# SensorsINI/Control_Toolkit

Hardware: AMD Instinct MI355X
Metric: trajectory-steps/sec (N*H per controller.step) (higher is better)
Workload: dtype f32; 1 GPU; MPPI N=1024 global (1024 per GPU), H=50, period=1, predictor ODE (4 states, 1 input) [mppi_cfg2]; boundary=controller_mpc.step (Python; s in, u out on the host), samples=buffer, global_rollouts=1024, parallelism=single GPU

## Files before the change

### control_toolkit_amd/Optimizers/optimizer_mppi_hip.py

```python
from typing import Tuple

import numpy as np

from . import template_optimizer, logging_kwargs
from ..computation_library import HipLibrary


class optimizer_mppi_hip(template_optimizer):
    supported_computation_libraries = (HipLibrary,)
    engine_name = "mppi"

    def __init__(self, predictor, cost_function, control_limits: "Tuple[np.ndarray, np.ndarray]",
                 computation_library, seed, cc_weight: float, R: float, LBD: float, mpc_horizon: int,
                 num_rollouts: int, NU: float, SQRTRHOINV: float, period_interpolation_inducing_points: int,
                 optimizer_logging: bool, calculate_optimal_trajectory: bool = False, **kwargs):
        super().__init__(predictor=predictor, cost_function=cost_function, control_limits=control_limits,
                         optimizer_logging=optimizer_logging, seed=seed, num_rollouts=num_rollouts,
                         mpc_horizon=mpc_horizon, computation_library=computation_library,
                         calculate_optimal_trajectory=calculate_optimal_trajectory,
                         rng_mode=kwargs.get("rng_mode", "device"), device=kwargs.get("device", 0), **logging_kwargs(kwargs))
        self.cc_weight, self.R, self.LBD, self.NU = cc_weight, R, LBD, NU
        self._SQRTRHOINV = SQRTRHOINV
        self.period_interpolation_inducing_points = period_interpolation_inducing_points
        self.global_rollout_offset = int(kwargs.get("global_rollout_offset", 0))
        self.resident_idle_us = float(kwargs.get("resident_idle_us", 0.0) or 0.0)

    def configure(self, num_states: int, num_control_inputs: int, dt: float, predictor_specification: str, **kwargs):
        super().configure(num_states=num_states, num_control_inputs=num_control_inputs, default_configure=False)
        self._build_engine(dt, predictor_specification, cc_weight=self.cc_weight, R=self.R, LBD=self.LBD, NU=self.NU,
                           SQRTRHOINV=self._SQRTRHOINV,
                           period_interpolation_inducing_points=self.period_interpolation_inducing_points,
                           global_rollout_offset=self.global_rollout_offset)
        self.number_of_interpolation_inducing_points = self.engine.inducing_points()
        if self.resident_idle_us > 0.0:
            self.engine.resident_enable(True, self.resident_idle_us)
        self.optimizer_reset()

    def step(self, s: np.ndarray, time=None):
        fast = self._fast
        if fast is not None:
            u = fast(s)
            if u is not NotImplemented:
                return u
        if self.optimizer_logging:
            self.logging_values = {"s_logged": np.asarray(s).copy()}
        s = self._prepare_state(s)
        self._sync_parameters()
        noise = self._draws("normal", [self.num_rollouts, self.number_of_interpolation_inducing_points, self.num_control_inputs])
        self._publish_u(self.engine.step(s, noise, u_prev=self._u_prev()))
        self._lazy.clear()
# ... 14 lines not shown
```

### control_toolkit_amd/_capi.py

```python
from __future__ import annotations

import ctypes as C
import os
from types import SimpleNamespace
from typing import NamedTuple, Optional

import numpy as np

_HERE = os.path.dirname(os.path.abspath(__file__))
_LIB_NAME = "libctk_hip.so"
_lib = None

OPTIMIZERS = {"mppi": 0, "cem": 1, "rpgd": 2, "random_action": 3, "gradient": 4, "cem_naive_grad": 5,
              "cem_grad_bharadhwaj": 6, "cem_gmm": 7}
PREDICTORS = {"ODE": 0, "MLP": 1, "GRU": 2}
ENVIRONMENTS = {"CartPole": 0, "Quad2D": 1, "Hover": 2}
MAX_STATES, MAX_INPUTS = 8, 4
PARAMS = ("g", "m_cart", "m_pole", "L", "u_max", "M_fric", "J_fric", "target_position", "target_equilibrium",
          "dd_weight", "ep_weight", "ekp_weight", "cc_weight", "ccrc_weight", "R", "x_scale", "terminal_weight")
BUFFERS = {"Q": 0, "J": 1, "TRAJ": 2, "U_NOM": 3, "STD": 4, "ADAM_M": 5, "ADAM_V": 6, "AGES": 7, "BEST_IDX": 8, "PLAN": 9, "AGES_LOGGED": 10,
           "MIX_MU": 11, "MIX_STD": 12, "MIX_PROB": 13, "MIX_LABEL": 14}
LOC_NONE, LOC_HOST, LOC_DEVICE = 0, 1, 2
MLP_NUM_WEIGHTS = 1380

# ... 168 lines not shown

HYPERS = {"cc_weight": 0, "R": 1, "LBD": 2, "NU": 3, "SQRTRHOINV": 4}
_PROBLEM_HYPER = {
    "set_hyper": (C.c_int, [_H, C.c_int, C.c_void_p, C.c_int, C.c_void_p]),
    "get_hyper": (C.c_int, [_H, C.c_int, C.c_int, _FP]),
    "set_limits": (C.c_int, [_H, C.c_int, C.c_void_p, C.c_void_p, C.c_void_p]),
    "get_limits": (C.c_int, [_H, C.c_int, C.c_void_p, C.c_void_p]),
    "hypers_differ": (C.c_int, [_H]),
}
HYPER_SYMBOLS = {}
for _batch, _problem in _BATCH_FAMILIES[:3]:
    HYPER_SYMBOLS.update({f"{_problem}_{name}": sig for name, sig in _PROBLEM_HYPER.items()})
    HYPER_SYMBOLS[f"{_batch}_set_hyper"] = (C.c_int, [_H, C.c_int, C.c_float])


USER_ENVIRONMENTS = {}
ENV_USER = 3
_user_libs = {}


def load_library(path: str = None):
    global _lib
    if path is not None:
        if path not in _user_libs:
            _user_libs[path] = _bind_library(path)
        return _user_libs[path]
    if _lib is not None:
        return _lib
    try:
        import torch
# ... 4 lines not shown


def _bind_library(path: str):
    try:
        import torch
    except ImportError:
        pass
    if not os.path.exists(path):
        raise CtkError(f"{path} not found: build it with `make -C control_toolkit_amd/csrc` "
                       f"(or `python -c 'import __graft_entry__ as g; g.build()'`). There is no CPU fallback.")
    try:
        lib = C.CDLL(path)
    except OSError as e:
        raise CtkError(f"cannot load {path}: {e}") from e
    for name, (res, args) in list(SYMBOLS.items()) + list(RUN_SYMBOLS.items()) + list(EPISODE_SYMBOLS.items()) + list(LOOP_SYMBOLS.items()) + \
            list(GRU_LOOP_SYMBOLS.items()) + list(HYPER_SYMBOLS.items()):
        fn = getattr(lib, name)
        fn.restype, fn.argtypes = res, args
    if lib.ctk_abi_version() != 6:
        raise CtkError(f"{path}: ABI version mismatch")
    return lib


def environment_library(name: str):
    if name in ENVIRONMENTS:
        return load_library(), ENVIRONMENTS[name]
    if name in USER_ENVIRONMENTS:
        return load_library(USER_ENVIRONMENTS[name]), ENV_USER
    raise NotImplementedError(f"environment {name!r} is not built (have: {sorted(ENVIRONMENTS)} + registered user environments "
                              f"{sorted(USER_ENVIRONMENTS)}; control_toolkit_amd.build_env.register_environment compiles a model header)")

# ... 387 lines not shown
        if name == "BEST_IDX":
            return out.astype(np.int64)
        return out.reshape(shapes[name])

    def resident_enable(self, on: bool = True, idle_us: float = 200.0, read_ahead: bool = False):
        self._check(self._lib.ctk_resident_enable(self._h, (2 if read_ahead else 1) if on else 0, float(idle_us)))

    def resident_stop(self):
        self._check(self._lib.ctk_resident_stop(self._h))

    def resident_stats(self) -> dict:
        a, b, r, m = C.c_uint64(0), C.c_uint64(0), C.c_int(0), C.c_int(0)
        self._check(self._lib.ctk_resident_stats(self._h, C.byref(a), C.byref(b), C.byref(r), C.byref(m)))
        return {"launches": int(a.value), "steps": int(b.value), "running": bool(r.value), "mailbox": "device memory" if m.value else "pinned host memory"}

    def log_enable(self, capacity_steps: int):
        self._check(self._lib.ctk_log_enable(self._h, int(capacity_steps)))
        self.log_capacity = int(capacity_steps)

    def log_count(self) -> int:
        return int(self._lib.ctk_log_count(self._h))

    def log_read(self, name: str, first_step: int, n_steps: int) -> np.ndarray:
        N, H = self.N, self.H
        shape = {"Q": (N, H, self.C), "J": (N,), "TRAJ": (N, H + 1, self.S), "AGES": (N,)}[name]
        out = np.empty((int(n_steps),) + shape, np.float32)
        n = C.c_size_t()
        self._check(self._lib.ctk_log_read(self._h, BUFFERS[name], int(first_step), int(n_steps), _ptr(out), out.size, C.byref(n)))
        assert n.value == out.size
        return out
# ... 882 lines not shown
```

### control_toolkit_amd/csrc/ctk_api.hip

```cpp
#include <atomic>
#include <unordered_map>
#include <chrono>
#include <cmath>
#include <cstdio>
#include <cstring>
#include <string>
#include <vector>

#include "ctk_launch.h"
#include "ctk_host.h"
#include "ctk_device.h"
#include "ctk_mlp.h"
#include "ctk_gru.h"
#include "ctk_env.h"
#include "ctk_net.h"
#include <algorithm>
#include <cstdlib>

thread_local std::string ctk_host::g_create_error;
using namespace ctk_host;

namespace {

struct EventPair {
// ... 103 lines not shown
    CtkResidentBox* res_box_dev = nullptr;
    bool res_local = false;
    bool res_stream_isolated = false;
    CtkResidentStat* res_stat = nullptr;
    CtkResidentStat* res_stat_dev = nullptr;
    CtkResidentBox* d_res_relay = nullptr;
    void* d_res_args = nullptr;
    alignas(16) unsigned char res_args_host[CTK_RES_ARGS_BYTES];
    uint32_t res_req = 0;
    uint32_t res_relay_prime[2] = {0, 0};
    uint64_t res_launches = 0, res_steps = 0;
    std::string res_dominant_saved;
    std::unordered_map<const float*, const float*> res_follow;
    const float* res_prev_samples = nullptr;
    bool res_readahead = false;
    Owner own;
    ~ctk_handle();
};

namespace {

int fail(ctk_handle* h, int code, const std::string& msg) {
    if (h) h->err = msg; else g_create_error = msg;
    return code;
}

#define HIP_TRY(h, expr)                                                                      \
    do {                                                                                      \
        hipError_t _e = (expr);                                                               \
        if (_e != hipSuccess)                                                                 \
// ... 538 lines not shown
        }
        return fail(h, CTK_ERR_STATE, dev_err == 1 ? "timed out waiting for a peer's record (a rank is gone or out of step)"
                                                   : "in-launch record hand-off timed out (a workgroup's record never arrived)");
    }
    return h->log_cap ? log_step(h) : CTK_OK;
}

template <class F>
int guarded(ctk_handle* h, F&& body) {
    const uint32_t seq0 = h->seq;
    const int rc = body();
    if (rc != CTK_OK && h->seq == seq0) ++h->seq;
    return rc;
}

int resident_quiesce(ctk_handle* h) {
    if (!h->res_running) return CTK_OK;
    if (__atomic_load_n(&h->res_stat->state, __ATOMIC_ACQUIRE) != CTK_RES_LEFT) {
        volatile CtkResidentBox* b = h->res_box;
        b->cmd = CTK_RES_CMD_EXIT;
        b->tail = h->res_req + 1;
        __builtin_ia32_sfence();
        b->req = ++h->res_req;
        __builtin_ia32_sfence();
    }
    HIP_TRY(h, hipStreamSynchronize(h->stream));
    h->res_running = false;
    if (!h->res_dominant_saved.empty()) { h->dominant = h->res_dominant_saved; h->res_dominant_saved.clear(); }
    return CTK_OK;
}
// ... 62 lines not shown
                if (*slot == want) break;
                if (int rc = resident_launch(h, req)) return rc;
            }
            if (std::chrono::duration<double>(std::chrono::steady_clock::now() - t0).count() > 5.0) {
                (void)resident_quiesce(h);
                return fail(h, CTK_ERR_HIP, "resident step: no result within 5 s");
            }
        }
        __builtin_ia32_pause();
    }
    ++h->res_steps;
    h->cur ^= 1;
    return finish_step(h, u_out);
}

#define RES_Q(h) do { if ((h) != nullptr && (h)->res_running) { const int _q = resident_quiesce(h); if (_q != CTK_OK) return _q; } } while (0)

int check_predictor(ctk_handle* h) {
    if (h->cfg.predictor != CTK_PRED_ODE && !h->have_weights)
        return fail(h, CTK_ERR_STATE, "network predictor: call ctk_set_predictor_weights before stepping");
    return CTK_OK;
}

int mppi_block_parts(const ctk_handle* h) {
    if (h->generic && h->cfg.predictor != CTK_PRED_ODE) return ctk_g_rollout_net_blocks(h->env, h->net, CTK_G_MODE_MPPI, h->N, h->P, h->H);
    return h->generic ? ctk_g_rollout_blocks(h->N) : ctk_mppi_num_blocks(h->N, h->cfg.predictor);
}
bool mppi_env_kernel(const ctk_handle* h) {
    return h->generic && h->cfg.predictor == CTK_PRED_ODE && !ctk_mppi_uses_throughput_kernel(CTK_PRED_ODE, h->N) &&
           ctk_mppi_rollout_env_lds(h->env, h->P, h->H, h->N) <= 160 * 1024;
}
// ... 25 lines not shown
        if (h->cfg.predictor != CTK_PRED_ODE)
            HIP_TRY(h, ctk_launch_g_rollout_net(h->stream, h->env, h->net, CTK_G_MODE_MPPI, a, h->params, h->cfg.dt, h->cfg.intermediate_steps,
                                                h->mk, d_s, h->d_unom[h->cur], nullptr, 0, h->d_wperm, h->d_parts, log, ps.a, ps.b, &fz));
        else
            HIP_TRY(h, ctk_launch_g_rollout(h->stream, h->env, CTK_G_MODE_MPPI, a, h->params, h->cfg.dt, h->cfg.intermediate_steps, h->mk, d_s,
                                            h->d_unom[h->cur], nullptr, 0, h->d_parts, log, ps.a, ps.b));
        return CTK_OK;
    }
    const char* ran = nullptr;
    CTK_HSTAMP(h, 1);
    HIP_TRY(h, ctk_launch_mppi_rollout(h->stream, h->cfg.predictor, a, h->k, h->mk, d_s, h->d_unom[h->cur], h->d_wperm,
                                       h->d_parts, log, fz, ps.a, ps.b, &ran));
    CTK_HSTAMP(h, 2);
    if (ran != h->dominant_ran) { h->dominant_ran = ran; h->dominant = ran; }
    return CTK_OK;
}

int mppi_reduce_blocks(ctk_handle* h, const float** parts, int* n_parts) {
    int n = mppi_block_parts(h);
    const float* src = h->d_parts;
    float* bufs[2] = {h->d_parts2, h->d_parts3};
    int b = 0;
    while (n > 64) {
        HIP_TRY(h, ctk_launch_mppi_merge_partial(h->stream, src, n, 32, h->PC, h->mk.neg_inv_lbd, bufs[b]));
        n = (n + 31) / 32;
        src = bufs[b];
        b ^= 1;
    }
    *parts = src; *n_parts = n;
    return CTK_OK;
// ... 321 lines not shown
    return CTK_OK;
}

int fill_const(ctk_handle* h, float* d, float v, int n) {
    std::vector<float> tmp((size_t)n, v);
    HIP_TRY(h, hipMemcpyAsync(d, tmp.data(), n * sizeof(float), hipMemcpyHostToDevice, h->stream));
    HIP_TRY(h, hipStreamSynchronize(h->stream));
    return CTK_OK;
}

}

inline ctk_handle::~ctk_handle() {
    if (!stream && own.empty() && events.empty() && p2p_world == 0) return;
    hipSetDevice(cfg.device);
    (void)resident_quiesce(this);
    hipStreamSynchronize(stream);
    for (auto& e : events) { hipEventDestroy(e.a); hipEventDestroy(e.b); }
    ctk_p2p_close(this);
    own.release();
    if (own_stream && stream) hipStreamDestroy(stream);
}

extern "C" {

int ctk_abi_version(void) { return CTK_ABI_VERSION; }
static_assert(CTK_P_COUNT <= CTK_MAX_PARAMS && CTK_Q_COUNT <= CTK_MAX_PARAMS && CTK_V_COUNT <= CTK_MAX_PARAMS, "parameter table size");
static_assert(Env<CTK_ENV_QUAD2D>::S <= CTK_MAX_STATES && Env<CTK_ENV_QUAD2D>::C <= CTK_MAX_INPUTS, "environment dimensions");
static_assert(Env<CTK_ENV_HOVER>::S <= CTK_MAX_STATES && Env<CTK_ENV_HOVER>::C <= CTK_MAX_INPUTS, "environment dimensions");

// ... 159 lines not shown
    const bool gnet = generic && cfg->predictor != CTK_PRED_ODE;
    if (descends) h->dominant = gnet ? ctk_g_rpgd_descent_net_name(h->env, h->net, (int)N, (int)H) : generic ? ctk_g_rpgd_descent_name(h->env) : ctk_rpgd_descent_name(cfg->predictor, (int)N, (int)H);
    else {
        const int mode = cfg->optimizer == CTK_OPT_MPPI ? CTK_G_MODE_MPPI : CTK_G_MODE_AFFINE;
        h->dominant = gnet ? ctk_g_rollout_net_name(h->env, h->net, mode, mat, (int)N, (int)P, (int)H) : generic ? ctk_g_rollout_name(h->env, mode, mat)
                    : cfg->optimizer == CTK_OPT_MPPI ? ctk_mppi_rollout_name(cfg->predictor, mat, cfg->num_rollouts, cfg->period_interpolation_inducing_points == 1 && h->P == (int)H, false)
                                                     : ctk_affine_rollout_name(cfg->predictor, mat);
    }
    if (h->d_cem_ll && h->variant == CTK_OPT_CEM && cfg->cem_best_k <= (int)N) h->dominant = ctk_cem_fused_name(h->env, mat);
    if (cfg->optimizer == CTK_OPT_MPPI && mppi_env_kernel(h)) h->dominant = ctk_mppi_rollout_env_name(h->env, mat);
    if (!descends && cfg->optimizer != CTK_OPT_MPPI && affine_env_kernel(h) && !(h->d_cem_ll && h->variant == CTK_OPT_CEM)) h->dominant = ctk_affine_rollout_env_name(h->env, mat);
    if (h->gmm_in_rollout) h->dominant = ctk_affine_rollout_mix_name(h->env, mat);
    if (cfg->optimizer != CTK_OPT_RPGD)
        if (int rc = ctk_reset(h, nullptr, CTK_LOC_NONE)) { g_create_error = h->err; return rc; }
    HIP_CREATE(hipStreamSynchronize(h->stream));
    *out = made.release();
    return CTK_OK;
}

void ctk_destroy(ctk_handle* h) { delete h; }


int ctk_set_stream(ctk_handle* h, void* hip_stream) {
    RES_Q(h);
    if (!h) return CTK_ERR_INVALID_ARGUMENT;
    HIP_TRY(h, hipSetDevice(h->cfg.device));
    hipStream_t ns = (hipStream_t)hip_stream;
    if (ns == h->stream) return CTK_OK;
    if (h->own_stream && h->stream) {
        HIP_TRY(h, hipStreamSynchronize(h->stream));
// ... 172 lines not shown
    else HIP_TRY(h, hipMemsetAsync(gru_hidden(h), 0, GRU_HIDDEN_FLOATS * sizeof(float), h->stream));
    HIP_TRY(h, hipStreamSynchronize(h->stream));
    return CTK_OK;
}

size_t ctk_samples_needed(const ctk_handle* h) { return h ? samples_needed(h) : 0; }

int ctk_rng_get_position(const ctk_handle* h, uint32_t* call) {
    if (!h || !call) return CTK_ERR_INVALID_ARGUMENT;
    *call = h->call;
    return CTK_OK;
}

int ctk_rng_set_position(ctk_handle* h, uint32_t call) {
    if (!h) return CTK_ERR_INVALID_ARGUMENT;
    h->call = call;
    return CTK_OK;
}

int ctk_step(ctk_handle* h, const float* s, const float* u_prev, const float* samples, int samples_loc, float* u_out) {
    if (!h || !s) return h ? fail(h, CTK_ERR_INVALID_ARGUMENT, "ctk_step: NULL state") : CTK_ERR_INVALID_ARGUMENT;
    CTK_HSTAMP(h, 0);
    return guarded(h, [&]() -> int {
    if (h->mppi_pending) return fail(h, CTK_ERR_STATE, "ctk_step: a sharded step is pending (call ctk_mppi_step_end)");
    HIP_TRY(h, hipSetDevice(h->cfg.device));
    switch (h->cfg.optimizer) {
        case CTK_OPT_MPPI: {
            for (int i = 0; i < h->S; ++i) h->mppi_s[i] = s[i];
            if (resident_ok(h, samples_loc)) {
                const float* d_s = nullptr;
                if (int rc = resolve_samples(h, samples, samples_loc, (size_t)h->N * h->PC, &d_s)) return rc;
                return resident_step(h, s, u_prev, d_s, u_out);
            }
            if (int rc = resident_quiesce(h)) return rc;
            if (mppi_can_fuse(h)) {
                if (int rc = mppi_rollout(h, s, u_prev, samples, samples_loc, 1, nullptr)) return rc;
                h->cur ^= 1;
                if (int rc = mppi_advance_hidden(h)) return rc;
                return finish_step(h, u_out);
            }
            if (int rc = mppi_rollout(h, s, u_prev, samples, samples_loc, 0, nullptr)) return rc;
            const float* parts; int n_parts;
            if (int rc = mppi_reduce_blocks(h, &parts, &n_parts)) return rc;
            return mppi_update(h, parts, n_parts, u_out);
        }
        case CTK_OPT_CEM: return cem_step(h, s, u_prev, samples, samples_loc, u_out);
        case CTK_OPT_RANDOM_ACTION: return random_step(h, s, u_prev, samples, samples_loc, u_out);
        case CTK_OPT_RPGD: return rpgd_step(h, s, u_prev, samples, samples_loc, u_out);
    }
// ... 458 lines not shown
                HIP_TRY(h, hipStreamSynchronize(h->stream));
                (void)hipStreamDestroy(h->stream);
                h->stream = ns;
            }
        }
        (void)hipGetLastError();
        h->res_stream_isolated = true;
    }
    h->res_idle_us = idle_us;
    h->res_readahead = on == 2;
    h->res_follow.clear(); h->res_prev_samples = nullptr;
    h->res_enabled = true;
    return CTK_OK;
}

int ctk_resident_stop(ctk_handle* h) {
    if (!h) return CTK_ERR_INVALID_ARGUMENT;
    HIP_TRY(h, hipSetDevice(h->cfg.device));
    return resident_quiesce(h);
}

int ctk_resident_stats(const ctk_handle* h, uint64_t* launches, uint64_t* steps, int* running, int* mailbox_in_device_memory) {
    if (!h) return CTK_ERR_INVALID_ARGUMENT;
    if (h->res_stat && getenv("CTK_RES_TRACE"))
        fprintf(stderr, "[ctk resident] mailbox in %s memory; last request: fetch%s %.2f us, block 0's step %.2f us, inputs %s\n", h->res_local ? "device" : "pinned host",
                h->res_local ? "" : " + relay", (h->res_stat->t_relay & 0x7FFFFFFFu) * 0.01, h->res_stat->t_body * 0.01,
                (h->res_stat->t_relay & 0x80000000u) ? "prepared ahead" : "formed at the request");
    if (h->res_stat && getenv("CTK_RES_TRACE"))
    {
        fprintf(stderr, "[ctk resident] block 0's step: %u shader cycles -> %.0f MHz; stamps", h->res_stat->c_body, h->res_stat->c_body / (h->res_stat->t_body * 0.01 + 1e-9));
        for (int i = 1; i < 12; ++i) fprintf(stderr, " %d", (int)(h->res_stat->stamps[i] - h->res_stat->stamps[0]));
        fprintf(stderr, "\n");
    }
    if (launches) *launches = h->res_launches;
// ... 66 lines not shown
```

### control_toolkit_amd/csrc/ctk_launch.h

```cpp
#pragma once
#include <hip/hip_ext.h>
#include "ctk_common.h"

#define CTK_LAUNCH(kernel, grid, block, lds, st, e0, e1, ...)                                         \
    do {                                                                                              \
        if (e0) hipExtLaunchKernelGGL(kernel, grid, block, lds, st, e0, e1, 0, __VA_ARGS__);          \
        else hipLaunchKernelGGL(kernel, grid, block, lds, st, __VA_ARGS__);                           \
    } while (0)

#include <type_traits>
template <class F>
inline void ctk_with_bool(bool b, F&& f) {
    if (b) f(std::true_type{});
    else f(std::false_type{});
}

inline RolloutArgs ctk_rollout_args(const RolloutArgs& a_in, int C, int cols) {
    RolloutArgs a = a_in;
    a.C = C; a.P = cols; a.p_magic = ctk_magic_of(cols);
    return a;
}
inline RolloutArgs ctk_descent_args(const RolloutArgs& a_in, int C) {
    RolloutArgs a = a_in;
    a.C = C; a.p_magic = ctk_magic_of(a.H * C);
// ... 76 lines not shown
};
hipError_t ctk_launch_mppi_rollout(hipStream_t st, int pred, const RolloutArgs& a, const EnvK& k, const MppiK& m,
                                   const float* samples, const float* u_nom, const float* wperm, float* parts, bool log,
                                   const MppiFuse& fuse, hipEvent_t ev_start = nullptr, hipEvent_t ev_stop = nullptr,
                                   const char** ran = nullptr);
hipError_t ctk_launch_mppi_rollout_env(hipStream_t st, int env, const float* params, float dt, int isteps, const RolloutArgs& a, const MppiK& m,
                                       const float* samples, const float* u_nom, float* parts, bool log, const MppiFuse& fuse,
                                       hipEvent_t ev_start = nullptr, hipEvent_t ev_stop = nullptr);
size_t ctk_mppi_rollout_env_lds(int env, int P, int H, int N);
hipError_t ctk_launch_mppi_resident(hipStream_t st, int env, const float* params, float dt, int isteps, const RolloutArgs& a, const MppiK& m,
                                    float* u_nom0, float* u_nom1, float* parts, const MppiFuse& fuse, const CtkResidentBox* box_dev, int box_local,
                                    CtkResidentStat* stat_dev, CtkResidentBox* relay, double idle_us, uint32_t first_req, void* args_dev, void* args_host);
constexpr size_t CTK_RES_ARGS_BYTES = 1024;
const char* ctk_mppi_resident_name(int env, int N, int P);
const char* ctk_mppi_rollout_env_name(int env, bool log);
struct CtkBatchDesc {
    float* parts;
    unsigned long long* ll;
    float* J;
    float* Q_out;
    float* traj_out;
    float* unom[2];
    float* u_dev;
    float* u_host;
    uint32_t seed_lo, seed_hi;
};
struct CtkBatchStep {
    int32_t id;
    uint32_t seq;
    uint32_t call;
// ... 322 lines not shown
```

### control_toolkit_amd/csrc/ctk_mppi.hip

```cpp
#ifdef CTK_STAMPS
#define STAMP(i)                                                                                   \
    do {                                                                                           \
        __builtin_amdgcn_sched_barrier(0);                                                         \
        unsigned long long _t;                                                                     \
        asm volatile("s_memtime %0\n\ts_waitcnt lgkmcnt(0)" : "=s"(_t)::"memory");                 \
        __builtin_amdgcn_sched_barrier(0);                                                         \
        if (threadIdx.x == 0 && a.stamps) a.stamps[blockIdx.x * 16 + (i)] = _t;                     \
    } while (0)
#else
#define STAMP(i)
#endif

#include "ctk_rollout.h"
#include "ctk_env.h"
#include "ctk_mlp.h"
#include "ctk_gru.h"
#include "ctk_launch.h"
#include "ctk_mppi_merge.h"
#include <cstring>
#include <type_traits>

constexpr int MPPI_TRAJ = 64;
constexpr int MPPI_WAVES = 4;
constexpr int MPPI_BLOCK = MPPI_TRAJ * MPPI_WAVES;
// ... 1099 lines not shown
    ctk_with_bool(log, [&](auto log_c) {
        hipLaunchKernelGGL((ctk_mppi_batch_mlp_hp<decltype(log_c)::value>), grid, block, lds, st, desc_dev, steps_dev, a.interp, w_dev, k_dev, a.N, a.H,
                           a.P, pmagic, wstride, a, fz);
    });
}
static void launch_batch_gru_hp(hipStream_t st, dim3 grid, dim3 block, size_t lds, const CtkBatchDesc* desc_dev, const CtkBatchStep* steps_dev, const float* w_dev,
                                const unsigned char* k_dev, uint32_t pmagic, uint32_t wstride, const RolloutArgs& a,
                                const FuseArgs& fz, bool log, int form) {
    with_mppi_form<false>(form, [&](auto form_c) {
        ctk_with_bool(log, [&](auto log_c) {
            hipLaunchKernelGGL((ctk_mppi_batch_gru_hp<decltype(log_c)::value, decltype(form_c)::value>), grid, block, lds, st, desc_dev, steps_dev,
                               a.interp, w_dev, k_dev, a.N, a.H, a.P, pmagic, wstride, a, fz);
        });
    });
}
```

### include/ctk_hip.h

```cpp
#ifndef CTK_HIP_H
#define CTK_HIP_H

#include <stddef.h>
#include <stdint.h>

#ifdef __cplusplus
extern "C" {
#endif

#define CTK_ABI_VERSION 6
#define CTK_MAX_STATES 8
#define CTK_MAX_INPUTS 4

typedef struct ctk_handle ctk_handle;

typedef enum ctk_status {
    CTK_OK = 0,
    CTK_ERR_INVALID_ARGUMENT = 1,
    CTK_ERR_UNSUPPORTED = 2,
    CTK_ERR_HIP = 3,
    CTK_ERR_NO_DEVICE = 4,
    CTK_ERR_STATE = 5
} ctk_status;

// ... 297 lines not shown
int ctk_gru_problem_set_weights(ctk_gru_batch* b, int n_ids, const int32_t* ids, const float* w, size_t n);
int ctk_gru_problem_have_weights(const ctk_gru_batch* b, int problem);
int ctk_gru_problem_get_hidden(ctk_gru_batch* b, int n_ids, const int32_t* ids, float* dst);
int ctk_gru_problem_set_hidden(ctk_gru_batch* b, int n_ids, const int32_t* ids, const float* src);
int ctk_gru_batch_fit(int num_rollouts, int mpc_horizon, int period_interpolation_inducing_points, int* blocks, int* record_words,
                      int* wide_tail, size_t* lds_bytes);

#ifdef __cplusplus
}
#endif
#include "ctk_hip_run.h"
#include "ctk_hip_episode.h"
#include "ctk_hip_loop.h"
#include "ctk_hip_gru.h"
#include "ctk_hip_hyper.h"
#endif
```

Baseline: 2.704 billion trajectory-steps/s.

## Pre-launch next MPPI step kernel that waits on a device-memory mailbox

Adds a launch-ahead path. After each MPPI step, once calls keep arriving in quick succession, the host enqueues the next step's fused rollout kernel in advance. That kernel spins on a fine-grained VRAM mailbox (large-BAR) until the host writes the new state and u_prev, then runs. If no request arrives within a fuse window, the kernel exits and the host falls back to a normal launch. This is meant to hide kernel launch latency from the per-step host boundary. The cost is added complexity, GPU spinning, and cancellation paths.

```diff
diff --git a/control_toolkit_amd/Optimizers/optimizer_mppi_hip.py b/control_toolkit_amd/Optimizers/optimizer_mppi_hip.py
--- a/control_toolkit_amd/Optimizers/optimizer_mppi_hip.py
+++ b/control_toolkit_amd/Optimizers/optimizer_mppi_hip.py
@@ -24,6 +24,7 @@
         self.period_interpolation_inducing_points = period_interpolation_inducing_points
         self.global_rollout_offset = int(kwargs.get("global_rollout_offset", 0))
         self.resident_idle_us = float(kwargs.get("resident_idle_us", 0.0) or 0.0)
+        self.launch_ahead = bool(kwargs.get("launch_ahead", True))
 
     def configure(self, num_states: int, num_control_inputs: int, dt: float, predictor_specification: str, **kwargs):
         super().configure(num_states=num_states, num_control_inputs=num_control_inputs, default_configure=False)
@@ -34,6 +35,8 @@
         self.number_of_interpolation_inducing_points = self.engine.inducing_points()
         if self.resident_idle_us > 0.0:
             self.engine.resident_enable(True, self.resident_idle_us)
+        if not self.launch_ahead:
+            self.engine.launch_ahead(False)
         self.optimizer_reset()
 
     def step(self, s: np.ndarray, time=None):
diff --git a/control_toolkit_amd/_capi.py b/control_toolkit_amd/_capi.py
--- a/control_toolkit_amd/_capi.py
+++ b/control_toolkit_amd/_capi.py
@@ -206,6 +206,25 @@
     HYPER_SYMBOLS[f"{_batch}_set_hyper"] = (C.c_int, [_H, C.c_int, C.c_float])
 
 
+class AheadRule(C.Structure):
+    _fields_ = [("streak", C.c_int32), ("armed", C.c_int32), ("untaken", C.c_int32), ("arms", C.c_int32)]
+
+
+class AheadCounters(C.Structure):
+    _fields_ = [("launched", C.c_uint64), ("taken", C.c_uint64), ("untaken", C.c_uint64), ("cancelled", C.c_uint64), ("arms", C.c_uint64),
+                ("armed", C.c_int32), ("pending", C.c_int32), ("available", C.c_int32), ("on", C.c_int32)]
+
+
+AHEAD_ARM_AFTER, AHEAD_DISARM_AFTER, AHEAD_DEFAULT_FUSE_US = 8, 2, 20.0
+AHEAD_NONE, AHEAD_TAKEN, AHEAD_UNTAKEN = 0, 1, 2
+AHEAD_SYMBOLS = {
+    "ctk_ahead_rule_step": (C.c_int, [C.POINTER(AheadRule), C.c_int, C.c_double, C.c_double, C.c_int]),
+    "ctk_ahead_enable": (C.c_int, [_H, C.c_int, C.c_double]),
+    "ctk_ahead_stats": (C.c_int, [_H, C.POINTER(AheadCounters), C.POINTER(C.c_double)]),
+    "ctk_ahead_kernel": (C.c_char_p, [_H]),
+}
+
+
 USER_ENVIRONMENTS = {}
 ENV_USER = 3
 _user_libs = {}
@@ -240,7 +259,7 @@
     except OSError as e:
         raise CtkError(f"cannot load {path}: {e}") from e
     for name, (res, args) in list(SYMBOLS.items()) + list(RUN_SYMBOLS.items()) + list(EPISODE_SYMBOLS.items()) + list(LOOP_SYMBOLS.items()) + \
-            list(GRU_LOOP_SYMBOLS.items()) + list(HYPER_SYMBOLS.items()):
+            list(GRU_LOOP_SYMBOLS.items()) + list(HYPER_SYMBOLS.items()) + list(AHEAD_SYMBOLS.items()):
         fn = getattr(lib, name)
         fn.restype, fn.argtypes = res, args
     if lib.ctk_abi_version() != 6:
@@ -658,6 +677,19 @@
         self._check(self._lib.ctk_resident_stats(self._h, C.byref(a), C.byref(b), C.byref(r), C.byref(m)))
         return {"launches": int(a.value), "steps": int(b.value), "running": bool(r.value), "mailbox": "device memory" if m.value else "pinned host memory"}
 
+    def launch_ahead(self, on: bool = True, fuse_us: float = 0.0):
+        self._check(self._lib.ctk_ahead_enable(self._h, 1 if on else 0, float(fuse_us)))
+
+    def ahead_stats(self) -> dict:
+        c, f = AheadCounters(), C.c_double()
+        self._check(self._lib.ctk_ahead_stats(self._h, C.byref(c), C.byref(f)))
+        out = {n: int(getattr(c, n)) for n, _ in AheadCounters._fields_}
+        out["fuse_us"] = f.value
+        return out
+
+    def ahead_kernel(self) -> str:
+        return (self._lib.ctk_ahead_kernel(self._h) or b"").decode()
+
     def log_enable(self, capacity_steps: int):
         self._check(self._lib.ctk_log_enable(self._h, int(capacity_steps)))
         self.log_capacity = int(capacity_steps)
diff --git a/control_toolkit_amd/csrc/ctk_api.hip b/control_toolkit_amd/csrc/ctk_api.hip
--- a/control_toolkit_amd/csrc/ctk_api.hip
+++ b/control_toolkit_amd/csrc/ctk_api.hip
@@ -141,6 +141,20 @@
     std::unordered_map<const float*, const float*> res_follow;
     const float* res_prev_samples = nullptr;
     bool res_readahead = false;
+    bool ah_on = true;
+    bool ah_avail = false;
+    bool ah_pending = false;
+    bool ah_have_result = false;
+    double ah_fuse_us = CTK_AHEAD_DEFAULT_FUSE_US;
+    CtkAheadBox* ah_box = nullptr;
+    uint32_t* ah_state = nullptr;
+    uint32_t* ah_state_dev = nullptr;
+    uint32_t* d_ah_relay = nullptr;
+    uint32_t ah_req = 0;
+    int ah_outcome = CTK_AHEAD_NONE;
+    ctk_ahead_rule ah_rule{};
+    std::chrono::steady_clock::time_point ah_t_result{};
+    uint64_t ah_launched = 0, ah_taken = 0, ah_untaken = 0, ah_cancelled = 0;
     Owner own;
     ~ctk_handle();
 };
@@ -709,6 +723,23 @@
     return rc;
 }
 
+int ahead_quiesce(ctk_handle* h) {
+    if (!h->ah_pending) return CTK_OK;
+    if (*const_cast<volatile uint32_t*>(h->ah_state) != ctk_ahead_state(h->ah_req, CTK_RES_LEFT)) {
+        volatile CtkAheadBox* b = h->ah_box;
+        b->cmd = CTK_RES_CMD_EXIT;
+        b->tail = h->ah_req;
+        __builtin_ia32_sfence();
+        b->req = h->ah_req;
+        __builtin_ia32_sfence();
+    }
+    h->ah_pending = false;
+    h->ah_outcome = CTK_AHEAD_NONE;
+    ++h->ah_cancelled;
+    HIP_TRY(h, hipStreamSynchronize(h->stream));
+    return CTK_OK;
+}
+
 int resident_quiesce(ctk_handle* h) {
     if (!h->res_running) return CTK_OK;
     if (__atomic_load_n(&h->res_stat->state, __ATOMIC_ACQUIRE) != CTK_RES_LEFT) {
@@ -801,7 +832,8 @@
     return finish_step(h, u_out);
 }
 
-#define RES_Q(h) do { if ((h) != nullptr && (h)->res_running) { const int _q = resident_quiesce(h); if (_q != CTK_OK) return _q; } } while (0)
+#define RES_Q(h) do { if ((h) != nullptr && (h)->ah_pending) { const int _a = ahead_quiesce(h); if (_a != CTK_OK) return _a; }                  \
+                      if ((h) != nullptr && (h)->res_running) { const int _q = resident_quiesce(h); if (_q != CTK_OK) return _q; } } while (0)
 
 int check_predictor(ctk_handle* h) {
     if (h->cfg.predictor != CTK_PRED_ODE && !h->have_weights)
@@ -857,6 +889,114 @@
     CTK_HSTAMP(h, 2);
     if (ran != h->dominant_ran) { h->dominant_ran = ran; h->dominant = ran; }
     return CTK_OK;
+}
+
+bool ahead_off_for_process() {
+    static const bool off = std::getenv("CTK_MPPI_NO_AHEAD") != nullptr;
+    return off;
+}
+
+void ahead_setup(ctk_handle* h) {
+    h->ah_avail = false;
+    if (const char* f = std::getenv("CTK_MPPI_AHEAD_FUSE_US")) { const double v = std::atof(f); if (v >= 1.0 && v <= 1.0e4) h->ah_fuse_us = v; }
+    if (ahead_off_for_process() || h->cfg.optimizer != CTK_OPT_MPPI || h->cfg.predictor != CTK_PRED_ODE || h->cfg.materialize_trajectories ||
+        !h->own_stream || h->d_ll == nullptr || !mppi_can_fuse(h) || (h->generic && !mppi_env_kernel(h)) ||
+        !ctk_mppi_ahead_ok(h->env, h->N, h->H, h->P))
+        return;
+    int large_bar = 0;
+    if (hipDeviceGetAttribute(&large_bar, hipDeviceAttributeIsLargeBar, h->cfg.device) != hipSuccess || !large_bar) { (void)hipGetLastError(); return; }
+    void* vram = nullptr;
+    if (hipExtMallocWithFlags(&vram, 4096, hipDeviceMallocFinegrained) != hipSuccess || !vram) { (void)hipGetLastError(); return; }
+    bool local = false;
+    if (hipMemset(vram, 0, 4096) == hipSuccess && hipDeviceSynchronize() == hipSuccess) {
+        volatile uint32_t* pv = static_cast<volatile uint32_t*>(vram);
+        for (int i = 0; i < 32; ++i) pv[i] = 0xA4EAD000u + (uint32_t)i;
+        __builtin_ia32_sfence();
+        uint32_t back[32] = {};
+        if (hipMemcpy(back, vram, sizeof(back), hipMemcpyDeviceToHost) == hipSuccess) {
+            local = true;
+            for (int i = 0; i < 32; ++i) local = local && back[i] == 0xA4EAD000u + (uint32_t)i;
+        }
+    }
+    if (!local || hipMemset(vram, 0, 4096) != hipSuccess || hipDeviceSynchronize() != hipSuccess) { (void)hipFree(vram); (void)hipGetLastError(); return; }
+    h->own.own_dev(vram);
+    h->ah_box = static_cast<CtkAheadBox*>(vram);
+    h->d_ah_relay = reinterpret_cast<uint32_t*>(static_cast<unsigned char*>(vram) + 2048);
+    if (h->own.pinned_zero(&h->ah_state, 64, hipHostMallocMapped | hipHostMallocCoherent) != hipSuccess ||
+        hipHostGetDevicePointer((void**)&h->ah_state_dev, h->ah_state, 0) != hipSuccess) { (void)hipGetLastError(); return; }
+    h->ah_avail = true;
+}
+
+bool ahead_eligible(const ctk_handle* h, int samples_loc) {
+    return h->ah_avail && h->ah_on && h->own_stream && samples_loc != CTK_LOC_HOST && h->log_cap == 0 && !h->prof && !h->mppi_pending &&
+           !h->res_enabled && !h->p2p_connected;
+}
+
+int ahead_launch(ctk_handle* h) {
+    float zs[CTK_MAX_STATES] = {};
+    RolloutArgs a = make_args(h, zs, nullptr, h->N, h->P);
+    a.call = h->call + 1u;
+    MppiFuse fz;
+    fz.mode = 1; fz.counter = h->d_counter; fz.ll = h->d_ll;
+    fz.u_nom_out = h->d_unom[h->cur ^ 1]; fz.u_dev = h->d_u; fz.u_host = h->h_u_dev; fz.seq = h->seq + 1u;
+    CtkAheadGate g{};
+    g.box = h->ah_box; g.state = h->ah_state_dev; g.relay = h->d_ah_relay; g.req = ++h->ah_req;
+    g.fuse_ticks = (unsigned long long)(h->ah_fuse_us * 100.0);
+    HIP_TRY(h, ctk_launch_mppi_ahead(h->stream, h->env, h->params, h->cfg.dt, h->cfg.intermediate_steps, a, h->mk, h->d_unom[h->cur], h->d_parts, fz, g));
+    h->ah_pending = true;
+    ++h->ah_launched;
+    return CTK_OK;
+}
+
+int ahead_step(ctk_handle* h, const float* s, const float* u_prev, const float* samples, int samples_loc, float* u_out) {
+    const auto t_in = std::chrono::steady_clock::now();
+    const double gap_us = h->ah_have_result ? std::chrono::duration<double, std::micro>(t_in - h->ah_t_result).count() : -1.0;
+    bool served = false;
+    if (h->ah_pending) {
+        const float* d_s = nullptr;
+        if (int rc = resolve_samples(h, samples, samples_loc, (size_t)h->N * h->PC, &d_s)) { (void)ahead_quiesce(h); return rc; }
+        volatile uint32_t* st = h->ah_state;
+        const uint32_t R = h->ah_req, taken = ctk_ahead_state(R, CTK_RES_RUNNING), left = ctk_ahead_state(R, CTK_RES_LEFT);
+        uint32_t seen = *st;
+        if (seen != left) {
+            volatile CtkAheadBox* b = h->ah_box;
+            b->cmd = CTK_RES_CMD_STEP; b->dev_uprev = u_prev ? 0u : 1u; b->samples = d_s;
+            for (int i = 0; i < h->S; ++i) b->s[i] = s[i];
+            for (int c = 0; c < h->C; ++c) b->u_prev[c] = u_prev ? u_prev[c] : 0.0f;
+            b->tail = R;
+            __builtin_ia32_sfence();
+            b->req = R;
+            __builtin_ia32_sfence();
+            CTK_HSTAMP(h, 1);
+            const auto t0 = std::chrono::steady_clock::now();
+            for (uint64_t spin = 1;; ++spin) {
+                seen = *st;
+                if (seen == taken || seen == left) break;
+                if ((spin & 4095) == 0 && std::chrono::duration<double>(std::chrono::steady_clock::now() - t0).count() > 2.0) {
+                    HIP_TRY(h, hipStreamSynchronize(h->stream));
+                    seen = *st;
+                    if (seen != taken) seen = left;
+                    break;
+                }
+                __builtin_ia32_pause();
+            }
+            CTK_HSTAMP(h, 2);
+        }
+        h->ah_pending = false;
+        served = seen == taken;
+        h->ah_outcome = served ? CTK_AHEAD_TAKEN : CTK_AHEAD_UNTAKEN;
+        if (served) ++h->ah_taken;
+        else { ++h->ah_untaken; ++h->seq; }
+    }
+    const bool armed = ctk_ahead_rule_step(&h->ah_rule, 1, gap_us, h->ah_fuse_us, h->ah_outcome) != 0;
+    h->ah_outcome = CTK_AHEAD_NONE;
+    if (!served) if (int rc = mppi_rollout(h, s, u_prev, samples, samples_loc, 1, nullptr)) return rc;
+    h->cur ^= 1;
+    if (armed) if (int rc = ahead_launch(h)) return rc;
+    const int rc = finish_step(h, u_out);
+    h->ah_t_result = std::chrono::steady_clock::now();
+    h->ah_have_result = true;
+    return rc;
 }
 
 int mppi_reduce_blocks(ctk_handle* h, const float** parts, int* n_parts) {
@@ -1208,6 +1348,11 @@
 inline ctk_handle::~ctk_handle() {
     if (!stream && own.empty() && events.empty() && p2p_world == 0) return;
     hipSetDevice(cfg.device);
+    if (ah_launched && std::getenv("CTK_AHEAD_TRACE"))
+        fprintf(stderr, "[ctk ahead] fuse %.0f us: launched %llu taken %llu untaken %llu cancelled %llu pending %d arms %d\n", ah_fuse_us,
+                (unsigned long long)ah_launched, (unsigned long long)ah_taken, (unsigned long long)ah_untaken, (unsigned long long)ah_cancelled,
+                ah_pending ? 1 : 0, (int)ah_rule.arms);
+    (void)ahead_quiesce(this);
     (void)resident_quiesce(this);
     hipStreamSynchronize(stream);
     for (auto& e : events) { hipEventDestroy(e.a); hipEventDestroy(e.b); }
@@ -1397,6 +1542,7 @@
     if (cfg->optimizer != CTK_OPT_RPGD)
         if (int rc = ctk_reset(h, nullptr, CTK_LOC_NONE)) { g_create_error = h->err; return rc; }
     HIP_CREATE(hipStreamSynchronize(h->stream));
+    ahead_setup(h);
     *out = made.release();
     return CTK_OK;
 }
@@ -1599,6 +1745,7 @@
 
 int ctk_rng_set_position(ctk_handle* h, uint32_t call) {
     if (!h) return CTK_ERR_INVALID_ARGUMENT;
+    RES_Q(h);
     h->call = call;
     return CTK_OK;
 }
@@ -1613,11 +1760,18 @@
         case CTK_OPT_MPPI: {
             for (int i = 0; i < h->S; ++i) h->mppi_s[i] = s[i];
             if (resident_ok(h, samples_loc)) {
+                if (int rc = ahead_quiesce(h)) return rc;
                 const float* d_s = nullptr;
                 if (int rc = resolve_samples(h, samples, samples_loc, (size_t)h->N * h->PC, &d_s)) return rc;
                 return resident_step(h, s, u_prev, d_s, u_out);
             }
             if (int rc = resident_quiesce(h)) return rc;
+            if (ahead_eligible(h, samples_loc)) return ahead_step(h, s, u_prev, samples, samples_loc, u_out);
+            if (h->ah_avail) {
+                if (int rc = ahead_quiesce(h)) return rc;
+                (void)ctk_ahead_rule_step(&h->ah_rule, 0, -1.0, h->ah_fuse_us, CTK_AHEAD_NONE);
+                h->ah_have_result = false;
+            }
             if (mppi_can_fuse(h)) {
                 if (int rc = mppi_rollout(h, s, u_prev, samples, samples_loc, 1, nullptr)) return rc;
                 h->cur ^= 1;
@@ -2106,10 +2260,48 @@
     return CTK_OK;
 }
 
+int ctk_ahead_rule_step(ctk_ahead_rule* r, int eligible, double gap_us, double fuse_us, int outcome) {
+    if (!r) return 0;
+    if (outcome == CTK_AHEAD_TAKEN) r->untaken = 0;
+    else if (outcome == CTK_AHEAD_UNTAKEN && ++r->untaken >= CTK_AHEAD_DISARM_AFTER) { r->armed = 0; r->streak = 0; r->untaken = 0; }
+    if (!eligible) { r->streak = 0; r->armed = 0; r->untaken = 0; return 0; }
+    if (gap_us >= 0.0 && gap_us <= fuse_us) { if (r->streak < CTK_AHEAD_ARM_AFTER) ++r->streak; }
+    else r->streak = 0;
+    if (!r->armed && r->streak >= CTK_AHEAD_ARM_AFTER) { r->armed = 1; r->untaken = 0; ++r->arms; }
+    return r->armed;
+}
+
+int ctk_ahead_enable(ctk_handle* h, int on, double fuse_us) {
+    if (!h) return CTK_ERR_INVALID_ARGUMENT;
+    RES_Q(h);
+    if (on != 0 && on != 1) return fail(h, CTK_ERR_INVALID_ARGUMENT, "ctk_ahead_enable: on must be 0 or 1");
+    if (fuse_us > 0.0 && !(fuse_us >= 1.0 && fuse_us <= 1.0e4)) return fail(h, CTK_ERR_INVALID_ARGUMENT, "ctk_ahead_enable: fuse_us must be within [1, 1e4] (<= 0 keeps the current value)");
+    if (fuse_us > 0.0) h->ah_fuse_us = fuse_us;
+    h->ah_on = on == 1 && !ahead_off_for_process();
+    h->ah_rule = ctk_ahead_rule{};
+    h->ah_have_result = false;
+    return CTK_OK;
+}
+
+const char* ctk_ahead_kernel(const ctk_handle* h) { return (h && h->ah_taken) ? ctk_mppi_ahead_name(h->env) : ""; }
+
+int ctk_ahead_stats(const ctk_handle* h, ctk_ahead_counters* out, double* fuse_us) {
+    if (!h) return CTK_ERR_INVALID_ARGUMENT;
+    if (out) {
+        *out = ctk_ahead_counters{};
+        out->launched = h->ah_launched; out->taken = h->ah_taken; out->untaken = h->ah_untaken; out->cancelled = h->ah_cancelled;
+        out->arms = (uint64_t)h->ah_rule.arms; out->armed = h->ah_rule.armed; out->pending = h->ah_pending ? 1 : 0;
+        out->available = h->ah_avail ? 1 : 0; out->on = (h->ah_on && !ahead_off_for_process()) ? 1 : 0;
+    }
+    if (fuse_us) *fuse_us = h->ah_fuse_us;
+    return CTK_OK;
+}
+
 int ctk_resident_stop(ctk_handle* h) {
     if (!h) return CTK_ERR_INVALID_ARGUMENT;
     HIP_TRY(h, hipSetDevice(h->cfg.device));
-    return resident_quiesce(h);
+    RES_Q(h);
+    return CTK_OK;
 }
 
 int ctk_resident_stats(const ctk_handle* h, uint64_t* launches, uint64_t* steps, int* running, int* mailbox_in_device_memory) {
diff --git a/control_toolkit_amd/csrc/ctk_launch.h b/control_toolkit_amd/csrc/ctk_launch.h
--- a/control_toolkit_amd/csrc/ctk_launch.h
+++ b/control_toolkit_amd/csrc/ctk_launch.h
@@ -114,6 +114,30 @@
 constexpr size_t CTK_RES_ARGS_BYTES = 1024;
 const char* ctk_mppi_resident_name(int env, int N, int P);
 const char* ctk_mppi_rollout_env_name(int env, bool log);
+struct alignas(128) CtkAheadBox {
+    uint32_t req;
+    uint32_t cmd;
+    uint32_t dev_uprev;
+    uint32_t pad;
+    const float* samples;
+    float s[CTK_MAX_STATES];
+    float u_prev[CTK_MAX_INPUTS];
+    uint32_t tail;
+};
+constexpr int CTK_AHEAD_BOX_WORDS = 19;
+constexpr uint32_t ctk_ahead_state(uint32_t req, uint32_t code) { return (req << 2) | code; }
+struct CtkAheadGate {
+    const CtkAheadBox* box;
+    uint32_t* state;
+    uint32_t* relay;
+    uint32_t req;
+    uint32_t pad;
+    unsigned long long fuse_ticks;
+};
+bool ctk_mppi_ahead_ok(int env, int N, int H, int P);
+const char* ctk_mppi_ahead_name(int env);
+hipError_t ctk_launch_mppi_ahead(hipStream_t st, int env, const float* params, float dt, int isteps, const RolloutArgs& a, const MppiK& m,
+                                 const float* u_nom, float* parts, const MppiFuse& fuse, const CtkAheadGate& gate);
 struct CtkBatchDesc {
     float* parts;
     unsigned long long* ll;
diff --git a/control_toolkit_amd/csrc/ctk_mppi.hip b/control_toolkit_amd/csrc/ctk_mppi.hip
--- a/control_toolkit_amd/csrc/ctk_mppi.hip
+++ b/control_toolkit_amd/csrc/ctk_mppi.hip
@@ -1137,3 +1137,103 @@
         });
     });
 }
+
+#define CTK_BODY_EARLY_U
+template <int ENV>
+__global__ __launch_bounds__(MPPI_BLOCK) void ctk_mppi_ahead(const CtkAheadBox* box, const float* __restrict__ u_nom,
+                                                             const InterpEntry* __restrict__ interp, const float* __restrict__ wperm,
+                                                             float* __restrict__ parts, int N_, int H_, int P_, uint32_t pmagic_,
+                                                             RolloutArgs a_tpl, typename Env<ENV>::K k, MppiK m, FuseArgs fz, CtkAheadGate g) {
+    constexpr int PRED = CTK_PRED_ODE, FORM = 0;
+    constexpr bool LOG = false, P2P = false;
+    constexpr int BOXW = CTK_AHEAD_BOX_WORDS, TAILW = BOXW - 1;
+    static_assert(offsetof(CtkAheadBox, req) == 0 && offsetof(CtkAheadBox, cmd) == 4 && offsetof(CtkAheadBox, tail) == 4 * TAILW && BOXW <= 64 &&
+                  sizeof(CtkAheadBox) == 128, "request layout");
+    extern __shared__ float lds[];
+    __shared__ uint32_t req_s[BOXW];
+    __shared__ int leave_s;
+    if (threadIdx.x < 64) {
+        const int gl = threadIdx.x;
+        const unsigned long long t0 = wall_clock64();
+        uint32_t w = 0;
+        auto look = [&]() {
+            const uint32_t x = gl < BOXW ? __hip_atomic_load(reinterpret_cast<const uint32_t*>(box) + gl, __ATOMIC_RELAXED, __HIP_MEMORY_SCOPE_SYSTEM) : 0u;
+            w = x;
+            return (uint32_t)__builtin_amdgcn_readlane((int)x, 0) == g.req && (uint32_t)__builtin_amdgcn_readlane((int)x, TAILW) == g.req;
+        };
+        auto state_store = [&](uint32_t v) { __hip_atomic_store(g.state, v, __ATOMIC_RELAXED, __HIP_MEMORY_SCOPE_SYSTEM); };
+        int leave = 0;
+        if (blockIdx.x == 0) {
+            for (;;) {
+                if (look()) break;
+                if (wall_clock64() - t0 > g.fuse_ticks) {
+                    if (gl == 0) { state_store(ctk_ahead_state(g.req, CTK_RES_LEAVING)); __threadfence_system(); }
+                    if (!look()) leave = 1;
+                    break;
+                }
+                __builtin_amdgcn_s_sleep(1);
+            }
+            if (!leave && (uint32_t)__builtin_amdgcn_readlane((int)w, 1) != (uint32_t)CTK_RES_CMD_STEP) leave = 1;
+            if (gl == 0) {
+                if (leave) {
+                    __hip_atomic_store(g.relay, g.req, __ATOMIC_RELEASE, __HIP_MEMORY_SCOPE_AGENT);
+                    state_store(ctk_ahead_state(g.req, CTK_RES_LEFT));
+                } else {
+                    state_store(ctk_ahead_state(g.req, CTK_RES_RUNNING));
+                }
+            }
+        } else {
+            leave = 1;
+            for (;;) {
+                if (look()) { leave = (uint32_t)__builtin_amdgcn_readlane((int)w, 1) != (uint32_t)CTK_RES_CMD_STEP ? 1 : 0; break; }
+                const uint32_t rr = gl == 0 ? __hip_atomic_load(g.relay, __ATOMIC_RELAXED, __HIP_MEMORY_SCOPE_AGENT) : 0u;
+                if ((uint32_t)__builtin_amdgcn_readfirstlane((int)rr) == g.req) break;
+                if (wall_clock64() - t0 > 4 * g.fuse_ticks + 100000ull) break;
+                __builtin_amdgcn_s_sleep(1);
+            }
+        }
+        if (gl < BOXW) req_s[gl] = w;
+        if (gl == 0) leave_s = leave;
+    }
+    __syncthreads();
+    if (leave_s) return;
+    __builtin_amdgcn_fence(__ATOMIC_ACQUIRE, "");
+    auto rq = [&](int i) { return (uint32_t)__builtin_amdgcn_readfirstlane((int)req_s[i]); };
+    RolloutArgs a_in = a_tpl;
+#pragma unroll
+    for (int i = 0; i < Env<ENV>::S; ++i) a_in.s0[i] = __builtin_bit_cast(float, rq(6 + i));
+#pragma unroll
+    for (int c = 0; c < Env<ENV>::C; ++c) a_in.u_prev[c] = __builtin_bit_cast(float, rq(14 + c));
+    if (rq(2) == 0u) a_in.u_prev_dev = nullptr;
+    const float* samples = reinterpret_cast<const float*>((unsigned long long)rq(4) | ((unsigned long long)rq(5) << 32));
+#include "ctk_mppi_body.inc"
+}
+#undef CTK_BODY_EARLY_U
+
+bool ctk_mppi_ahead_ok(int env, int N, int H, int P) {
+    if (N < 1 || ctk_mppi_uses_throughput_kernel(CTK_PRED_ODE, N) || mppi_late_u()) return false;
+    bool ok = false;
+    CTK_FOR_ENV(env, EV, {
+        const int blocks = (N + MPPI_TRAJ - 1) / MPPI_TRAJ;
+        int stage_ok;
+        const size_t lds = rollout_launch_lds(P, H, CTK_PRED_ODE, N, blocks, &stage_ok, Env<EV>::C);
+        ok = stage_ok != 0 && mppi_env_form<EV>(blocks, P * Env<EV>::C, true) == 0 && lds + 256 <= 160 * 1024;
+    });
+    return ok;
+}
+const char* ctk_mppi_ahead_name(int env) { return ctk_kernel_name("ctk_mppi_ahead<%d>", env); }
+
+hipError_t ctk_launch_mppi_ahead(hipStream_t st, int env, const float* params, float dt, int isteps, const RolloutArgs& a, const MppiK& m,
+                                 const float* u_nom, float* parts, const MppiFuse& fuse, const CtkAheadGate& gate) {
+    const dim3 grid((a.N + MPPI_TRAJ - 1) / MPPI_TRAJ), block(MPPI_BLOCK);
+    CTK_FOR_ENV(env, EV, {
+        using E = Env<EV>;
+        int stage_ok;
+        const size_t lds = rollout_launch_lds(a.P, a.H, CTK_PRED_ODE, a.N, (int)grid.x, &stage_ok, E::C);
+        if (!stage_ok || fuse.ll == nullptr || fuse.mode != 1) return hipErrorInvalidValue;
+        const FuseArgs fz = mppi_fuse_args(fuse, stage_ok, a, E::C, u_nom, fuse.u_nom_out);
+        hipLaunchKernelGGL((ctk_mppi_ahead<EV>), grid, block, lds, st, gate.box, u_nom, a.interp, static_cast<const float*>(nullptr), parts, a.N, a.H, a.P,
+                           ctk_magic_of(a.P * E::C), a, E::derive(params, dt, isteps), m, fz, gate);
+    });
+    return hipGetLastError();
+}
diff --git a/include/ctk_hip.h b/include/ctk_hip.h
--- a/include/ctk_hip.h
+++ b/include/ctk_hip.h
@@ -335,4 +335,5 @@
 #include "ctk_hip_loop.h"
 #include "ctk_hip_gru.h"
 #include "ctk_hip_hyper.h"
+#include "ctk_hip_ahead.h"
 #endif
diff --git a/include/ctk_hip_ahead.h b/include/ctk_hip_ahead.h
--- /dev/null
+++ b/include/ctk_hip_ahead.h
@@ -0,0 +1,39 @@
+#ifndef CTK_HIP_AHEAD_H
+#define CTK_HIP_AHEAD_H
+#include "ctk_hip.h"
+#ifdef __cplusplus
+extern "C" {
+#endif
+
+#define CTK_AHEAD_ARM_AFTER 8
+#define CTK_AHEAD_DISARM_AFTER 2
+enum ctk_ahead_outcome { CTK_AHEAD_NONE = 0, CTK_AHEAD_TAKEN = 1, CTK_AHEAD_UNTAKEN = 2 };
+typedef struct ctk_ahead_rule {
+    int32_t streak;
+    int32_t armed;
+    int32_t untaken;
+    int32_t arms;
+} ctk_ahead_rule;
+int ctk_ahead_rule_step(ctk_ahead_rule* r, int eligible, double gap_us, double fuse_us, int outcome);
+
+typedef struct ctk_ahead_counters {
+    uint64_t launched;
+    uint64_t taken;
+    uint64_t untaken;
+    uint64_t cancelled;
+    uint64_t arms;
+    int32_t armed;
+    int32_t pending;
+    int32_t available;
+    int32_t on;
+} ctk_ahead_counters;
+
+#define CTK_AHEAD_DEFAULT_FUSE_US 20.0
+int ctk_ahead_enable(ctk_handle* h, int on, double fuse_us);
+int ctk_ahead_stats(const ctk_handle* h, ctk_ahead_counters* out, double* fuse_us);
+const char* ctk_ahead_kernel(const ctk_handle* h);
+
+#ifdef __cplusplus
+}
+#endif
+#endif
```

After: 3.244 billion trajectory-steps/s, median of 6. +19.9%, better.
